# JdeRobot/slam-SDVL

Hardware: AMD Instinct MI355X
Metric: tracked frames/sec (640x480, 5-lvl pyr, ~200 feats) (higher is better)
Workload: dtype u8/f32/f64

## Files before the change

### include/sdvl_hip.h

```cpp
#ifndef SDVL_HIP_H_
#define SDVL_HIP_H_

#include <stdint.h>

#ifdef __cplusplus
extern "C" {
#endif

typedef struct sdvl_ctx sdvl_ctx;
typedef struct sdvl_frame sdvl_frame;

enum sdvl_status {
  SDVL_OK = 0,
  SDVL_ERR_INVALID = -1,
  SDVL_ERR_HIP = -2,
  SDVL_ERR_CAPACITY = -3,
  SDVL_ERR_NO_DEVICE = -4
};

#define SDVL_MAX_LEVELS 8
#define SDVL_MAX_CORNERS 6144
#define SDVL_MAX_ALIGN_FEATURES 2048
#define SDVL_CELL_KP_CAP 176
#define SDVL_MAX_CELL_SIZE 64
// ... 61 lines not shown
  int pad_;
} sdvl_search_params;

typedef struct sdvl_search_req {
  const sdvl_frame *cur;
  const sdvl_frame *ref;
  double cur_pose[7], ref_pose[7];
  double px[2];
  double bearing[3];
  double idepth, idepth_std;
  double px0[2];
  int32_t level;
  int32_t fixed;
  uint8_t desc[32];
} sdvl_search_req;

typedef struct sdvl_search_res {
  double px[2];
  int32_t found;
  int32_t level;
  int32_t best_corner;
  int32_t stage;
  int32_t lk_its;
  int32_t slevel;
} sdvl_search_res;

int sdvl_ctx_create(int device, sdvl_ctx **out);
int sdvl_ctx_destroy(sdvl_ctx *ctx);
const char *sdvl_last_error(const sdvl_ctx *ctx);
int sdvl_ctx_synchronize(sdvl_ctx *ctx);
// ... 282 lines not shown
} sdvl_track_point_stat;

int sdvl_track_create(sdvl_ctx *ctx, int n_trackers, int max_points, int max_features, int grid_cells, int max_matches,
                      int max_ransac_its, sdvl_track_set **out);
int sdvl_track_destroy(sdvl_ctx *ctx, sdvl_track_set *set);
int sdvl_frame_register(sdvl_ctx *ctx, const sdvl_frame *frame, const double *pose7);
int sdvl_frames_register(sdvl_ctx *ctx, int n, const sdvl_frame *const *frames, const double *poses7);
int sdvl_track_upload(sdvl_ctx *ctx, sdvl_track_set *set, int n, const int32_t *trackers, const int32_t *feat_buf, const int32_t *n_points,
                      const sdvl_track_point *points, const int32_t *n_features, const sdvl_track_feature *features);
int sdvl_track_append(sdvl_ctx *ctx, sdvl_track_set *set, int n, const int32_t *trackers, const int32_t *feat_buf, const int32_t *n_points,
                      const sdvl_track_point *points, const int32_t *n_features, const sdvl_track_feature *features);
int sdvl_track_align(sdvl_ctx *ctx, sdvl_track_set *set, int n_jobs, const sdvl_track_job *jobs, const uint16_t *cell_rank,
                     const int32_t *rand_raw, const sdvl_camera *cam, const sdvl_track_params *p);
int sdvl_track_search(sdvl_ctx *ctx, sdvl_track_set *set);
int sdvl_track_collect(sdvl_ctx *ctx, sdvl_track_set *set, int n_jobs, sdvl_track_result *results);
const sdvl_track_feature_out *sdvl_track_features(const sdvl_track_set *set, int job);
const sdvl_track_point_stat *sdvl_track_stats(const sdvl_track_set *set, int job);

struct sdvl_synth_view;
int sdvl_synth_render(sdvl_ctx *ctx, int n, const struct sdvl_synth_view *views, int width, int height,
                      void *dev_out, int64_t frame_bytes);
int sdvl_device_malloc(sdvl_ctx *ctx, int64_t bytes, void **out);
int sdvl_device_free(sdvl_ctx *ctx, void *p);
int sdvl_device_download(sdvl_ctx *ctx, const void *dev, int64_t bytes, void *host);
int sdvl_ctx_fork_mark(sdvl_ctx *ctx);
int sdvl_ctx_fork_begin(sdvl_ctx *ctx);
int sdvl_ctx_fork_end(sdvl_ctx *ctx);
int sdvl_host_alloc_pinned(sdvl_ctx *ctx, int64_t bytes, void **out);
int sdvl_host_free_pinned(sdvl_ctx *ctx, void *p);
int sdvl_host_register(sdvl_ctx *ctx, void *p, int64_t bytes);
// ... 7 lines not shown
```

### slam-sdvl_amd/__init__.py

```python
import ctypes as C
import os

import numpy as np

try:
    import torch
except ImportError:
    torch = None

_HERE = os.path.dirname(os.path.abspath(__file__))
CSRC = os.path.join(_HERE, "csrc")
LIB_PATH = os.path.join(CSRC, "libsdvl_hip.so")
HOST_LIB_PATH = os.path.join(_HERE, "host", "libsdvl_host.so")

SDVL_GRAY8, SDVL_RGB8, SDVL_BGR8, SDVL_RGBA8, SDVL_BGRA8 = 0, 1, 2, 3, 4

MAX_LEVELS = 8
MAX_CORNERS = 6144

u8p = C.POINTER(C.c_uint8)
i32p = C.POINTER(C.c_int32)
f64p = C.POINTER(C.c_double)
f32p = C.POINTER(C.c_float)

# ... 80 lines not shown
                ("R", C.c_double * 9), ("t", C.c_double * 3), ("plane", C.c_double * 4),
                ("seed", C.c_uint32), ("frame_id", C.c_uint32), ("texture", C.c_uint32), ("reserved_", C.c_uint32),
                ("dist", C.c_double * 5)]


ABI_SYMBOLS = [
    "sdvl_ctx_create", "sdvl_ctx_destroy", "sdvl_last_error", "sdvl_ctx_synchronize", "sdvl_ctx_stream",
    "sdvl_ctx_bind_thread", "sdvl_ctx_device", "sdvl_pointer_device", "sdvl_ctx_scratch_device",
    "sdvl_ctx_timing_enable", "sdvl_ctx_timing_only", "sdvl_ctx_timing_get", "sdvl_ctx_timing_reset",
    "sdvl_frame_create", "sdvl_frame_create_many", "sdvl_frame_destroy", "sdvl_frame_upload", "sdvl_frames_upload", "sdvl_ctx_prefetch_images", "sdvl_ctx_prefetch_fence", "sdvl_frame_set_image_device", "sdvl_frame_borrow_image_device",
    "sdvl_pyramid_build", "sdvl_frame_download_level", "sdvl_fast_num_cells", "sdvl_cell_kp_cap", "sdvl_fast_cells",
    "sdvl_detect_corners", "sdvl_frames_corner_counts", "sdvl_frame_download_corners", "sdvl_retain_best",
    "sdvl_frame_set_corners", "sdvl_frames_set_corners", "sdvl_frame_num_corners", "sdvl_shi_tomasi", "sdvl_orb_describe",
    "sdvl_frame_download_descriptors", "sdvl_filter_inputs", "sdvl_filter_inputs_begin", "sdvl_filter_inputs_end", "sdvl_filter_corners_begin", "sdvl_filter_corners_end", "sdvl_orb_describe_points", "sdvl_hamming_argmin", "sdvl_image_align", "sdvl_image_align_begin", "sdvl_image_align_end", "sdvl_align_store_create", "sdvl_align_store_destroy", "sdvl_align_store_write", "sdvl_image_align_begin_stored", "sdvl_search_points", "sdvl_search_begin", "sdvl_search_slot", "sdvl_search_run", "sdvl_align_patches", "sdvl_pose_from_matches", "sdvl_search_points_filter", "sdvl_search_run_filter", "sdvl_search_run_chain", "sdvl_search_chain_end", "sdvl_frame_footprint", "sdvl_undistort", "sdvl_frames_upload_undistorted", "sdvl_convert_gray", "sdvl_frames_upload_color", "sdvl_ctx_set_wait_hook", "sdvl_ctx_wait_done", "sdvl_ctx_wait_block", "sdvl_ctx_health", "sdvl_ctx_counters",
    "sdvl_track_create", "sdvl_track_destroy", "sdvl_frame_register", "sdvl_frames_register", "sdvl_track_upload", "sdvl_track_append", "sdvl_track_align", "sdvl_track_search",
    "sdvl_track_collect", "sdvl_track_features", "sdvl_track_stats",
    "sdvl_synth_render", "sdvl_device_malloc", "sdvl_device_free", "sdvl_device_download",
    "sdvl_frames_own_images", "sdvl_feed_create", "sdvl_feed_destroy", "sdvl_feed_last_error", "sdvl_feed_slot_arrived", "sdvl_feed_images", "sdvl_ctx_feed_acquire", "sdvl_ctx_feed_release", "sdvl_frame_footprint_cap", "sdvl_ctx_set_corner_capacity", "sdvl_frame_corner_capacity", "sdvl_detect_scratch_bytes",
    "sdvl_ctx_set_wait_spin", "sdvl_ctx_fork_mark", "sdvl_ctx_fork_begin", "sdvl_ctx_fork_end", "sdvl_host_alloc_pinned", "sdvl_host_free_pinned", "sdvl_host_register", "sdvl_host_unregister",
]

_lib = None


def load_library():
    global _lib
    if _lib is None:
        if not os.path.exists(LIB_PATH):
            raise SdvlError("libsdvl_hip.so is not built (%s): run `python -c 'import __graft_entry__ as g; g.build()'`"
                            % LIB_PATH)
        lib = C.CDLL(LIB_PATH)
# ... 551 lines not shown
```

### slam-sdvl_amd/csrc/sdvl_internal.h

```cpp
#ifndef SDVL_INTERNAL_H_
#define SDVL_INTERNAL_H_

#include <hip/hip_runtime.h>
#include <stdlib.h>
#include <hip/hip_ext.h>
#include <stdint.h>
#include <stdio.h>
#include <string.h>

#include <string>
#include <vector>

#include "../../include/sdvl_hip.h"

struct FrameView {
  uint8_t *level[SDVL_MAX_LEVELS];
  int32_t lw[SDVL_MAX_LEVELS], lh[SDVL_MAX_LEVELS];
  int32_t levels;
  int32_t n_corners;
  int32_t *corner_hdr;
  int32_t *corners;
  uint8_t *desc;
};

// ... 50 lines not shown
  void *d_detect = nullptr; size_t d_detect_bytes = 0;
  size_t pack_lds_limit = 0;
  int corner_cap = SDVL_MAX_CORNERS;
  size_t stage_off = 0;
  void *h_search = nullptr; size_t h_search_bytes = 0;
  void *d_search = nullptr; size_t d_search_bytes = 0;
  uint64_t search_busy_gen = ~0ull;
  void *d_registry = nullptr;
  int registry_cap = 0, registry_next = 0;
  std::vector<int> registry_free;
  void *d_counts = nullptr; size_t d_counts_bytes = 0;
  std::vector<sdvl_frame *> detect_frames;
  void *h_counts = nullptr; size_t h_counts_bytes = 0;
  uint64_t wait_gen = 0, counts_gen = ~0ull;
  long long counters[4] = {0, 0, 0, 0};
  std::vector<void *> slabs;
  volatile uint32_t *h_flag = nullptr;
  uint32_t flag_seq = 0;
  int wait_spin_us = 0;
  uint32_t align_ticket = 0;
  int align_pending = 0;
  uint32_t chain_ticket = 0;
  uint32_t filter_ticket = 0;
  int filter_pending = 0, filter_ccap = 0, filter_desc = 0;
  size_t filter_sc_bytes = 0, filter_row = 0;
  int chain_pending = 0;
  size_t chain_host_off = 0;
  int chain_obs_total = 0;
  void *d_nits = nullptr;
  std::vector<int32_t> nits_host;
// ... 70 lines not shown
```

### slam-sdvl_amd/csrc/sdvl_search.hip

```cpp
#include <unordered_map>
#include <utility>
#include <type_traits>
#include <vector>

#include <cmath>

#include "sdvl_internal.h"
#include "sdvl_math.h"
#include "sdvl_orb_device.h"
#include "sdvl_search_types.h"
#include "sdvl_search_prepare.h"

namespace {

using namespace sdvl;

struct PatchJob {
  const uint8_t *img;
  int w, h;
  double u, v;
};

constexpr bool kSearchOrbWindow = false, kSearchLkWindow = false;
constexpr int kLkWin = 20, kLkWinBack = 9;
// ... 203 lines not shown
#else
#define SDVL_STAT(i, v) do { } while (0)
#endif

#ifdef SDVL_SEARCH_STAMPS
__device__ unsigned long long *g_search_stamps;
constexpr int kStampRequests = 1 << 18;
#define SS_STAMP(k) do { const unsigned long long now_ = __builtin_amdgcn_s_memtime(); st_[k] += now_ - t_last_; t_last_ = now_; } while (0)
#define SS_FLUSH() do { if (lane == 0 && ri < kStampRequests && g_search_stamps) { for (int q_ = 0; q_ < 7; q_++) g_search_stamps[ri * 8 + q_] += st_[q_]; g_search_stamps[ri * 8 + 7] += 1ull; } } while (0)
#else
#define SS_STAMP(k) do { } while (0)
#define SS_FLUSH() do { } while (0)
#endif


template <bool kStage, int kW>
__global__ __launch_bounds__(64 * kW) __attribute__((amdgpu_waves_per_eu(8, 8))) void search_points_kernel(const SearchReqDev *__restrict__ reqs,
                                                                            const SearchFramePose *__restrict__ table,
                                                                            const SearchBlock *__restrict__ blocks,
                                                                            const SearchPrep *__restrict__ prep, Cam cam,
                                                                            sdvl_search_params prm, int n_blocks,
                                                                            sdvl_search_res *__restrict__ out,
                                                                            sdvl_search_res *__restrict__ out_host) {
  static_assert(kW == kWavesPerBlock || (kW == 1 && !kStage), "one wave per workgroup only without the shared corner stage");
  constexpr bool kOrbWindow = kSearchOrbWindow, kLkWindow = kSearchLkWindow;
  __shared__ WaveLds s_lds[kW];
  __shared__ uint32_t s_corners[kStage ? kLdsCorners : 1];
  const int lane = threadIdx.x & 63;
#ifdef SDVL_SEARCH_STAMPS
  unsigned long long st_[7] = {0, 0, 0, 0, 0, 0, 0}, t_last_ = __builtin_amdgcn_s_memtime();
#endif
  const int wv = kW == 1 ? static_cast<int>((blockIdx.x >> 3) % kWavesPerBlock) : __builtin_amdgcn_readfirstlane(static_cast<int>(threadIdx.x >> 6));
  const int per_xcd = static_cast<int>((kW == 1 ? gridDim.x / kWavesPerBlock : gridDim.x) >> 3);
  const int bi = static_cast<int>(blockIdx.x & 7u) * per_xcd + static_cast<int>(kW == 1 ? (blockIdx.x >> 3) / kWavesPerBlock : (blockIdx.x >> 3));
  if (bi >= n_blocks) return;
  const SearchBlock blk = blocks[bi];
  if (blk.count <= 0) return;
  const SearchFramePose &tcur = table[reqs[blk.first].cur];
  const int n_corners = min(tcur.f.n_ptr[0], SDVL_MAX_CORNERS);
  const int4 *corners_g = reinterpret_cast<const int4 *>(tcur.f.corners);
  const auto pack_corner = [](const int4 c) {
    return static_cast<uint32_t>(c.x) | (static_cast<uint32_t>(c.y) << 12) | (static_cast<uint32_t>(c.z) << 24);
  };
  const bool binned = tcur.f.bin_start != nullptr;
  if (kStage && !binned) {
    for (int ci = threadIdx.x; ci < min(n_corners, kLdsCorners); ci += 64 * kW) s_corners[ci] = pack_corner(corners_g[ci]);
    __syncthreads();
  }
  const auto corner_at = [&](int ci) { return (kStage && !binned && ci < kLdsCorners) ? s_corners[ci] : pack_corner(corners_g[ci]); };
  if (wv >= blk.count) return;
  const int ri = blk.first + wv;
  WaveLds &L = s_lds[kW == 1 ? 0 : wv];
  const SearchReqDev &rq = reqs[ri];
  const SearchFramePose &tref = table[rq.ref];
  sdvl_search_res res;
  res.px[0] = rq.px0[0];
  res.px[1] = rq.px0[1];
  res.found = 0;
  res.level = -1;
  res.best_corner = -1;
  res.stage = 0;
  res.lk_its = 0;
  res.slevel = -1;

  const int level = rq.level;
  const SearchPrep pr = prep[ri];
  if (!pr.alive) {
    if (lane == 0) { out[ri] = res; if (out_host) out_host[ri] = res; }
    return;
  }
  const auto epi = [&]() {
    const SearchPrep *pe = prep + ri;
    asm volatile("" : "+s"(pe));
    return pe;
  };
  const int slevel = pr.slevel;
  res.slevel = slevel;
  SS_STAMP(0);
  {
    const double I00 = pr.I00, I01 = pr.I01, I10 = pr.I10, I11 = pr.I11;
    const uint8_t *img = tref.f.level[level];
    const int W = tref.f.lw[level], H = tref.f.lh[level];
    const double pyrx = __builtin_ldexp(rq.px[0], -level), pyry = __builtin_ldexp(rq.px[1], -level);
    const bool bad = (I00 != I00);
// ... 230 lines not shown
  }
  SS_STAMP(2);
  res.stage = 1;
  bool matched = false;
  int best_ci = -1;
  if (best != ~0ull) {
    const int bscore = static_cast<int>(static_cast<unsigned>(best >> 20)) - 0x40000000;
    if (bscore < threshold + 1 && !(bscore >= threshold)) {
      matched = true;
      best_ci = static_cast<int>(best & 0xFFFFF);
    }
  }
  if (!matched) {
    if (lane == 0) { out[ri] = res; if (out_host) out_host[ri] = res; }
    SS_FLUSH();
    return;
  }
  res.best_corner = best_ci;
  const uint32_t bpk = best_pk;
  const int bx = static_cast<int>(bpk & 0xFFFu), by = static_cast<int>((bpk >> 12) & 0xFFFu), bl = static_cast<int>(bpk >> 24);
  const double mpx = static_cast<double>(bx * (1 << bl)), mpy = static_cast<double>(by * (1 << bl));
  res.px[0] = mpx;
  res.px[1] = mpy;
  float u = static_cast<float>(__builtin_ldexp(mpx, -slevel)), v = static_cast<float>(__builtin_ldexp(mpy, -slevel));
  int its = 0;
  const bool conv = kLkWindow ? align_patch_wave<true>(L, tcur.f.level[slevel], tcur.f.lw[slevel], tcur.f.lh[slevel], prm.max_align_its, lane, &u, &v,
                                                       &its, prm.lk_tree_sums != 0)
                              : align_patch_wave<false>(L, tcur.f.level[slevel], tcur.f.lw[slevel], tcur.f.lh[slevel], prm.max_align_its, lane, &u, &v,
                                                        &its, prm.lk_tree_sums != 0);
  SS_STAMP(4);
#ifdef SDVL_SEARCH_STAMPS
  st_[5] += its;
#endif
  res.lk_its = its;
  res.stage = 2;
  if (conv) {
    res.px[0] = static_cast<double>(u) * (1 << slevel);
    res.px[1] = static_cast<double>(v) * (1 << slevel);
    res.level = slevel;
    res.found = 1;
    res.stage = 3;
  }
  if (lane == 0) { out[ri] = res; if (out_host) out_host[ri] = res; }
  SS_FLUSH();
}

#ifdef SDVL_SEARCH_STAMPS
extern "C" int sdvl_debug_search_stamps(unsigned long long *out8, int reset) {
  static unsigned long long *d_buf = nullptr;
  const size_t bytes = sizeof(unsigned long long) * 8 * kStampRequests;
  if (reset) {
    if (!d_buf && hipMalloc(&d_buf, bytes) != hipSuccess) return -1;
    if (hipMemset(d_buf, 0, bytes) != hipSuccess) return -1;
    return hipMemcpyToSymbol(HIP_SYMBOL(g_search_stamps), &d_buf, sizeof(d_buf)) == hipSuccess ? 0 : -1;
  }
  if (!d_buf) return -1;
  std::vector<unsigned long long> h(static_cast<size_t>(8) * kStampRequests);
  if (hipMemcpy(h.data(), d_buf, bytes, hipMemcpyDeviceToHost) != hipSuccess) return -1;
  for (int q = 0; q < 8; q++) out8[q] = 0;
// ... 277 lines not shown
#ifdef SDVL_SEARCH_STATS
  {
    static int launches = 0;
    if (++launches % 200 == 0) {
      unsigned long long h[8];
      if (hipMemcpyFromSymbol(h, HIP_SYMBOL(g_search_stats), sizeof(h)) == hipSuccess)
        fprintf(stderr, "search stats after %d launches: requests %llu, binned %llu, full scans %llu (frame binned %llu, line ok %llu), scan rounds %llu, corners in range %llu\n",
                launches, h[0], h[1], h[2], h[6], h[7], h[3], h[4]);
    }
  }
#endif
  SDVL_HIP_CHECK(ctx, hipGetLastError());
  return SDVL_OK;
}

int sdvl_select_matches_launch(sdvl_ctx *ctx, int n_frames, const ChainFrameDev *d_frames, const int32_t *d_cand_req,
                               const int32_t *d_cand_first, const sdvl_search_res *d_res, const double *d_req_point,
                               const sdvl_camera *cam, PoseJobDev *d_jobs, sdvl_pose_obs *d_obs, int32_t *d_nobs, int32_t *d_match_cand) {
  if (n_frames <= 0) return SDVL_OK;
  Cam c{cam->width, cam->height, cam->fx, cam->fy, cam->u0, cam->v0};
  SDVL_LAUNCH(ctx, "select_matches", select_matches_kernel, dim3(n_frames), dim3(256), d_frames, d_cand_req, d_cand_first, d_res, d_req_point, c,
              d_jobs, d_obs, d_nobs, d_match_cand);
  SDVL_HIP_CHECK(ctx, hipGetLastError());
  return SDVL_OK;
}

extern "C" {

static_assert(sizeof(sdvl_search_req_packed) == sizeof(SearchReqDev), "public and device request records are one layout");

// ... 403 lines not shown
```

### slam-sdvl_amd/csrc/sdvl_search_types.h

```cpp
#ifndef SDVL_SEARCH_TYPES_H_
#define SDVL_SEARCH_TYPES_H_

#include "sdvl_internal.h"
#include "sdvl_math.h"

constexpr int kWavesPerBlock = 4;
constexpr int kLdsCorners = 4096;

struct SearchBlock {
  int first, count;
};

struct SearchFrame {
  const uint8_t *level[SDVL_MAX_LEVELS];
  int lw[SDVL_MAX_LEVELS], lh[SDVL_MAX_LEVELS];
  const int32_t *corners;
  const uint8_t *desc;
  const int32_t *n_ptr;
  int levels;
  int bin_gw;
  const int32_t *bin_start;
  const uint2 *bin_entries;
  int bin_cells, pad_;
  int pad2_[2];
};

// ... 65 lines not shown
  int cur_id, last_id;
  int frame_id, max_matches;
  int n_feat, n_points;
  double last_pose[7];
  double pad_;
  const uint8_t *last_level[SDVL_MAX_LEVELS];
  double T0[7];
  double pad2_;
};

extern "C" TrackPoint *sdvl_track_points_device(sdvl_track_set *set, int *max_points, int *n_trackers);

int sdvl_search_launch_device(sdvl_ctx *ctx, int n_slots, const SearchReqDev *d_reqs, const SearchFramePose *d_table,
                              const SearchBlock *d_blocks, int n_blocks, const sdvl_camera *cam, const sdvl_search_params *p,
                              SearchPrep *d_prep, sdvl_search_res *d_res, sdvl_search_res *h_res, bool prepared = false);
int sdvl_select_matches_launch(sdvl_ctx *ctx, int n_frames, const ChainFrameDev *d_frames, const int32_t *d_cand_req,
                               const int32_t *d_cand_first, const sdvl_search_res *d_res, const double *d_req_point,
                               const sdvl_camera *cam, PoseJobDev *d_jobs, sdvl_pose_obs *d_obs, int32_t *d_nobs, int32_t *d_match_cand);
int sdvl_image_align_track_enqueue(sdvl_ctx *ctx, int n_jobs, const TrackJobDev *d_jobs, const TrackPoint *d_points, const TrackFeat *d_feats0,
                                   const TrackFeat *d_feats1, int np, int nfeat_cap, int max_nf, int levels, const sdvl_camera *cam,
                                   const sdvl_align_params *p, sdvl_align_result *d_results, int batch_size);
extern "C" int sdvl_ensure_nits_table(sdvl_ctx *ctx, int npoints_cfg, int max_its, int max_size);

#endif
```

### slam-sdvl_amd/csrc/sdvl_track.hip

```cpp
#include <atomic>
#include <chrono>
#include <vector>

#include "sdvl_internal.h"
#include "sdvl_math.h"
#include "sdvl_search_types.h"
#include "sdvl_search_prepare.h"

namespace {

using namespace sdvl;


struct UploadRec {
  int tracker, feat_buf;
  int n_points, n_feat;
  long long point_off, feat_off;
  int point_dst, feat_dst;
  long long pad_;
};

struct RegisterRec {
  SearchFramePose e;
  int id, pad_;
// ... 46 lines not shown
  const int fw = r.n_feat * static_cast<int>(sizeof(TrackFeat) / 16);
  for (int i = threadIdx.x; i < fw; i += 256) df[i] = sf[i];
}

constexpr int kProjThreads = 512;

__global__ __launch_bounds__(kProjThreads) void track_project_kernel(const TrackJobDev *__restrict__ jobs, TrackPoint *__restrict__ points,
                                                                     const TrackFeat *__restrict__ feats0, const TrackFeat *__restrict__ feats1,
                                                                     int np, int nf, int stride, int mm, int max_its,
                                                                     const sdvl_align_result *__restrict__ ares,
                                                                     const uint16_t *__restrict__ cell_rank, int cells, Cam cam, int cell_size,
                                                                     int patch, SearchFramePose *__restrict__ registry,
                                                                     SearchReqDev *__restrict__ reqs, double *__restrict__ req_point,
                                                                     int32_t *__restrict__ cand_first, int32_t *__restrict__ cand_feat,
                                                                     SearchBlock *__restrict__ blocks, ChainFrameDev *__restrict__ chain,
                                                                     sdvl_search_params sprm, SearchPrep *__restrict__ prep) {
  extern __shared__ __attribute__((aligned(16))) uint8_t s_dyn[];
  unsigned long long *s_key = reinterpret_cast<unsigned long long *>(s_dyn);
  double *s_px = reinterpret_cast<double *>(s_key + stride);
  uint16_t *s_cell = reinterpret_cast<uint16_t *>(s_px + 2 * static_cast<size_t>(stride));
  __shared__ double s_pose[7];
  __shared__ int s_ncand;
  const int j = blockIdx.x, tid = threadIdx.x;
  const TrackJobDev &jb = jobs[j];
  const TrackFeat *F = (jb.feat_buf ? feats1 : feats0) + static_cast<size_t>(jb.tracker) * nf;
  TrackPoint *P = points + static_cast<size_t>(jb.tracker) * np;
  const int n_feat = jb.n_feat;
  const int base = j * stride;
  if (tid == 0) {
    const Rigid pose = se3_mul(se3_from7(ares[j].T), se3_from7(jb.last_pose));
    se3_to7(pose, s_pose);
// ... 60 lines not shown
    for (int w = 0; w < 8; w++) rq.desc[w] = p.desc[w];
    reqs[base + r] = rq;
    if (prep) prep[base + r] = search_prepare_one(rq, pose, se3_from7(registry[p.ref].pose), cam, sprm, &jb.cur);
    double *rp = req_point + 3 * static_cast<size_t>(base + r);
    rp[0] = p.P[0]; rp[1] = p.P[1]; rp[2] = p.P[2];
    cand_feat[base + r] = i;
    s_cell[r] = static_cast<uint16_t>(key >> 48);
  }
  __syncthreads();
  for (int k = tid; k < stride; k += static_cast<int>(blockDim.x)) {
    if (k < n_cand) {
      int first = k;
      const uint16_t c = s_cell[k];
      while (first > 0 && s_cell[first - 1] == c) first--;
      cand_first[base + k] = base + first;
    } else {
      reqs[base + k].level = -1;
      if (prep) {
        prep[base + k].alive = 0;
        prep[base + k].slevel = -1;
      }
    }
  }
  const int nblk = stride / kWavesPerBlock;
  for (int b = tid; b < nblk; b += static_cast<int>(blockDim.x)) {
    int cnt = n_cand - b * kWavesPerBlock;
    cnt = cnt < 0 ? 0 : (cnt > kWavesPerBlock ? kWavesPerBlock : cnt);
    blocks[j * nblk + b] = SearchBlock{base + b * kWavesPerBlock, cnt};
  }
  if (tid == 0) {
    ChainFrameDev c;
// ... 181 lines not shown
  int n, np, nf, cells, mm, max_its;
  TrackPoint *d_points = nullptr;
  TrackFeat *d_feats[2] = {nullptr, nullptr};
  uint8_t *d_scratch = nullptr;
  size_t scratch_bytes = 0;
  TrackJobDev *d_jobs;
  uint16_t *d_cell_rank;
  int32_t *d_rand;
  sdvl_align_result *d_ares;
  SearchReqDev *d_reqs;
  SearchPrep *d_prep;
  sdvl_search_res *d_res;
  double *d_reqpt;
  int32_t *d_cfirst, *d_cfeat;
  SearchBlock *d_blocks;
  ChainFrameDev *d_chain;
  PoseJobDev *d_pjobs;
  sdvl_pose_obs *d_obs;
  void *d_hyp;
  sdvl_pose_result *d_pres;
  int32_t *d_lists, *d_nobs;
  uint8_t *h_pinned = nullptr;
  sdvl_track_result *h_results;
  sdvl_track_feature_out *h_feats;
  sdvl_track_point_stat *h_stats;
  std::vector<int> n_points;
  std::vector<int> n_feat[2];
  std::vector<sdvl_track_job> jobs;
  int stride = 0;
  int phase = 0;
  uint32_t ticket = 0;
  sdvl_camera cam;
  sdvl_track_params prm;
};

namespace {
template <typename T>
T *carve(uint8_t *&p, size_t count) {
  T *r = reinterpret_cast<T *>(p);
  p += (sizeof(T) * count + 255) / 256 * 256;
  return r;
}
}

extern "C" {

int sdvl_track_create(sdvl_ctx *ctx, int n, int max_points, int max_features, int grid_cells, int max_matches, int max_ransac_its,
                      sdvl_track_set **out) {
// ... 1 lines not shown
  *out = nullptr;
  SDVL_REQUIRE(ctx, n >= 1 && n <= 65536, "tracker count out of range");
  SDVL_REQUIRE(ctx, max_points >= 1 && max_points < SDVL_TRACK_DUPLICATE && max_features >= 4 && max_features <= 4096, "table capacities out of range (features <= 4096)");
  SDVL_REQUIRE(ctx, grid_cells >= 1 && grid_cells <= 65535, "grid too large");
  SDVL_REQUIRE(ctx, max_matches >= 1 && max_matches <= 1024 && max_matches <= max_features, "max_matches outside the device pose stage's range (1024)");
  SDVL_REQUIRE(ctx, max_ransac_its >= 1 && max_ransac_its <= 4096, "bad max_ransac_its");
  SDVL_HIP_CHECK(ctx, sdvl_bind_device(ctx));
  sdvl_track_set *s = new sdvl_track_set();
  s->ctx = ctx;
  s->n = n;
  s->np = max_points;
  s->nf = (max_features + 3) / 4 * 4;
  s->cells = grid_cells;
  s->mm = max_matches;
  s->max_its = max_ransac_its;
  const size_t N = static_cast<size_t>(n), NF = N * s->nf;
  hipError_t e = hipMalloc(reinterpret_cast<void **>(&s->d_points), sizeof(TrackPoint) * N * s->np);
  if (e == hipSuccess) e = hipMalloc(reinterpret_cast<void **>(&s->d_feats[0]), sizeof(TrackFeat) * NF);
  if (e == hipSuccess) e = hipMalloc(reinterpret_cast<void **>(&s->d_feats[1]), sizeof(TrackFeat) * NF);
  for (int pass = 0; pass < 2 && e == hipSuccess; pass++) {
    uint8_t *p = pass ? s->d_scratch : nullptr;
    s->d_jobs = carve<TrackJobDev>(p, N);
    s->d_cell_rank = carve<uint16_t>(p, N * s->cells);
    s->d_rand = carve<int32_t>(p, N * s->max_its);
    s->d_ares = carve<sdvl_align_result>(p, N);
    s->d_reqs = carve<SearchReqDev>(p, NF);
    s->d_prep = carve<SearchPrep>(p, NF);
    s->d_res = carve<sdvl_search_res>(p, NF);
    s->d_reqpt = carve<double>(p, NF * 3);
    s->d_cfirst = carve<int32_t>(p, NF);
    s->d_cfeat = carve<int32_t>(p, NF);
    s->d_blocks = carve<SearchBlock>(p, NF / kWavesPerBlock);
    s->d_chain = carve<ChainFrameDev>(p, N);
    s->d_pjobs = carve<PoseJobDev>(p, N);
    s->d_obs = carve<sdvl_pose_obs>(p, N * s->mm);
    s->d_hyp = carve<uint8_t>(p, sdvl_pose_hyp_bytes() * N * s->max_its);
    s->d_pres = carve<sdvl_pose_result>(p, N);
    s->d_lists = carve<int32_t>(p, N * s->mm);
    s->d_nobs = carve<int32_t>(p, N);
    if (!pass) {
      s->scratch_bytes = reinterpret_cast<size_t>(p);
      e = hipMalloc(reinterpret_cast<void **>(&s->d_scratch), s->scratch_bytes);
    }
  }
  if (e == hipSuccess) {
    const size_t hb = (sizeof(sdvl_track_result) * N + 255) / 256 * 256, fb = (sizeof(sdvl_track_feature_out) * NF + 255) / 256 * 256;
    const size_t sb = sizeof(sdvl_track_point_stat) * N * s->np;
// ... 1 lines not shown
    if (e == hipSuccess) {
      memset(s->h_pinned, 0, hb + fb + sb);
      s->h_results = reinterpret_cast<sdvl_track_result *>(s->h_pinned);
      s->h_feats = reinterpret_cast<sdvl_track_feature_out *>(s->h_pinned + hb);
      s->h_stats = reinterpret_cast<sdvl_track_point_stat *>(s->h_pinned + hb + fb);
    }
  }
  if (e != hipSuccess) {
    ctx->err = std::string("sdvl_track_create: ") + hipGetErrorString(e);
    sdvl_track_destroy(ctx, s);
    return SDVL_ERR_HIP;
  }
  s->n_points.assign(n, 0);
  s->n_feat[0].assign(n, 0);
  s->n_feat[1].assign(n, 0);
  *out = s;
  return SDVL_OK;
}

TrackPoint *sdvl_track_points_device(sdvl_track_set *set, int *max_points, int *n_trackers) {
  if (max_points) *max_points = set->np;
  if (n_trackers) *n_trackers = set->n;
  return set->d_points;
}

int sdvl_track_destroy(sdvl_ctx *ctx, sdvl_track_set *s) {
  if (!ctx || !s) return SDVL_ERR_INVALID;
  (void)sdvl_bind_device(ctx);
  (void)sdvl_stream_wait(ctx);
  if (s->d_points) (void)hipFree(s->d_points);
  if (s->d_feats[0]) (void)hipFree(s->d_feats[0]);
  if (s->d_feats[1]) (void)hipFree(s->d_feats[1]);
  if (s->d_scratch) (void)hipFree(s->d_scratch);
  if (s->h_pinned) (void)hipHostFree(s->h_pinned);
  delete s;
  return SDVL_OK;
}

int sdvl_frame_register(sdvl_ctx *ctx, const sdvl_frame *f, const double *pose7) { return sdvl_frames_register(ctx, 1, &f, pose7); }

int sdvl_frames_register(sdvl_ctx *ctx, int n, const sdvl_frame *const *frames, const double *poses7) {
  if (!ctx || n < 0 || (n > 0 && (!frames || !poses7))) return SDVL_ERR_INVALID;
  if (n == 0) return SDVL_OK;
  for (int i = 0; i < n; i++)
    SDVL_REQUIRE(ctx, frames[i] && frames[i]->home == ctx && frames[i]->reg_id >= 0 && frames[i]->reg_id < ctx->registry_cap,
                 "frame was not created on this context");
  void *hs = nullptr, *dsx = nullptr;
  int rc = sdvl_stage_alloc(ctx, sizeof(RegisterRec) * static_cast<size_t>(n), &hs, &dsx);
  if (rc) return rc;
// ... 187 lines not shown
      SDVL_HIP_CHECK(ctx, hipFuncSetAttribute(reinterpret_cast<const void *>(track_project_kernel), hipFuncAttributeMaxDynamicSharedMemorySize,
                                              4096 * (8 + 16 + 2) + 64));
      attr_devices.fetch_or(bit, std::memory_order_release);
    }
  }
  {
    const size_t lds = static_cast<size_t>(stride) * (8 + 16 + 2) + 64;
    hipEvent_t ev_a = nullptr, ev_b = nullptr;
    sdvl_timer_events(ctx, "track_project", &ev_a, &ev_b);
    const int proj_threads = stride <= 256 ? (s->n > 32 ? 128 : 256) : kProjThreads;
    hipExtLaunchKernelGGL(track_project_kernel, dim3(n_jobs), dim3(proj_threads), lds, ctx->stream, ev_a, ev_b, 0,
                          static_cast<const TrackJobDev *>(s->d_jobs), s->d_points, static_cast<const TrackFeat *>(s->d_feats[0]),
                          static_cast<const TrackFeat *>(s->d_feats[1]), s->np, s->nf, stride, s->mm, s->max_its,
                          static_cast<const sdvl_align_result *>(s->d_ares), static_cast<const uint16_t *>(s->d_cell_rank), s->cells, c,
                          s->prm.cell_size, s->prm.patch_size, registry, s->d_reqs, s->d_reqpt, s->d_cfirst, s->d_cfeat, s->d_blocks, s->d_chain,
                          s->prm.search, s->d_prep);
    SDVL_HIP_CHECK(ctx, hipGetLastError());
  }
  int rc = sdvl_search_launch_device(ctx, n_jobs * stride, s->d_reqs, registry, s->d_blocks, n_jobs * (stride / kWavesPerBlock), &s->cam,
                                     &s->prm.search, s->d_prep, s->d_res, nullptr,  true);
  if (rc) return rc;
  rc = sdvl_select_matches_launch(ctx, n_jobs, s->d_chain, nullptr, s->d_cfirst, s->d_res, s->d_reqpt, &s->cam, s->d_pjobs, s->d_obs, s->d_nobs,
                                  nullptr);
  if (rc) return rc;
  sdvl_pose_params pp = s->prm.pose;
  pp.pad_ = 1;
  rc = sdvl_pose_enqueue_device(ctx, n_jobs, s->d_pjobs, s->d_obs, s->d_rand, static_cast<const int32_t *>(ctx->d_nits), &pp, s->d_hyp, s->d_pres,
                                s->d_lists, s->mm, s->n);
  if (rc) return rc;
  {
    const size_t lds = (static_cast<size_t>(stride + 1) * 2 + stride + 64 + 7) / 8 * 8 + static_cast<size_t>(s->mm) * 8;
    hipEvent_t ev_a = nullptr, ev_b = nullptr;
    sdvl_timer_events(ctx, "track_commit", &ev_a, &ev_b);
    hipExtLaunchKernelGGL(track_commit_kernel, dim3(n_jobs), dim3(256), lds, ctx->stream, ev_a, ev_b, 0, static_cast<const TrackJobDev *>(s->d_jobs),
                          s->d_points, static_cast<const TrackFeat *>(s->d_feats[0]), static_cast<const TrackFeat *>(s->d_feats[1]), s->d_feats[0],
// ... 12 lines not shown
int sdvl_track_collect(sdvl_ctx *ctx, sdvl_track_set *s, int n_jobs, sdvl_track_result *results) {
  if (!ctx || !s || s->ctx != ctx || !results) return SDVL_ERR_INVALID;
  SDVL_REQUIRE(ctx, s->phase == 2 && n_jobs == static_cast<int>(s->jobs.size()), "sdvl_track_collect without a matching sdvl_track_search");
  SDVL_HIP_CHECK(ctx, sdvl_mark_wait(ctx, SDVL_MARK_CHAIN, s->ticket));
  s->phase = 0;
  memcpy(results, s->h_results, sizeof(sdvl_track_result) * n_jobs);
  for (int j = 0; j < n_jobs; j++) {
    const sdvl_track_job &a = s->jobs[j];
    s->n_feat[1 - a.feat_buf][a.tracker] = results[j].matches;
    if (results[j].n_corners >= 0) a.cur->v.n_corners = results[j].n_corners;
  }
  ctx->wait_gen++;
  return SDVL_OK;
}

const sdvl_track_feature_out *sdvl_track_features(const sdvl_track_set *s, int job) {
  return (s && job >= 0 && job < s->n) ? s->h_feats + static_cast<size_t>(job) * s->nf : nullptr;
}

const sdvl_track_point_stat *sdvl_track_stats(const sdvl_track_set *s, int job) {
  return (s && job >= 0 && job < s->n) ? s->h_stats + static_cast<size_t>(job) * s->np : nullptr;
}

}
```

Before: 459,500.

## Search each grid cell's candidates sequentially in one wave, stopping at first match

The projection kernel now emits per-cell runs of candidate requests. A new search kernel assigns one wave per run and walks the candidates in order, breaking at the first converged match. It marks the remaining candidates as not tried instead of searching every candidate in parallel, which is meant to skip redundant searches whose results the per-cell match selection would discard. In exchange, work within a cell becomes serialised, and the kernel gives up the multi-wave blocks with the shared LDS corner stage. It is enabled only when there are more than 32 trackers, and an environment variable can turn it off. Host mirror and cell-inspection APIs are also added for checking results.

```diff
diff --git a/include/sdvl_hip.h b/include/sdvl_hip.h
--- a/include/sdvl_hip.h
+++ b/include/sdvl_hip.h
@@ -99,6 +99,8 @@
   int32_t fixed;
   uint8_t desc[32];
 } sdvl_search_req;
+
+#define SDVL_SEARCH_NOT_TRIED 4
 
 typedef struct sdvl_search_res {
   double px[2];
@@ -411,6 +413,8 @@
                      const int32_t *rand_raw, const sdvl_camera *cam, const sdvl_track_params *p);
 int sdvl_track_search(sdvl_ctx *ctx, sdvl_track_set *set);
 int sdvl_track_collect(sdvl_ctx *ctx, sdvl_track_set *set, int n_jobs, sdvl_track_result *results);
+int sdvl_track_search_mirror(sdvl_ctx *ctx, sdvl_track_set *set, int fill_byte, const sdvl_search_res **out, int *stride);
+int sdvl_track_search_cells(sdvl_ctx *ctx, sdvl_track_set *set, int job, int cap, int32_t *cand_first, int32_t *n_cand);
 const sdvl_track_feature_out *sdvl_track_features(const sdvl_track_set *set, int job);
 const sdvl_track_point_stat *sdvl_track_stats(const sdvl_track_set *set, int job);
 
diff --git a/slam-sdvl_amd/__init__.py b/slam-sdvl_amd/__init__.py
--- a/slam-sdvl_amd/__init__.py
+++ b/slam-sdvl_amd/__init__.py
@@ -118,7 +118,7 @@
     "sdvl_frame_set_corners", "sdvl_frames_set_corners", "sdvl_frame_num_corners", "sdvl_shi_tomasi", "sdvl_orb_describe",
     "sdvl_frame_download_descriptors", "sdvl_filter_inputs", "sdvl_filter_inputs_begin", "sdvl_filter_inputs_end", "sdvl_filter_corners_begin", "sdvl_filter_corners_end", "sdvl_orb_describe_points", "sdvl_hamming_argmin", "sdvl_image_align", "sdvl_image_align_begin", "sdvl_image_align_end", "sdvl_align_store_create", "sdvl_align_store_destroy", "sdvl_align_store_write", "sdvl_image_align_begin_stored", "sdvl_search_points", "sdvl_search_begin", "sdvl_search_slot", "sdvl_search_run", "sdvl_align_patches", "sdvl_pose_from_matches", "sdvl_search_points_filter", "sdvl_search_run_filter", "sdvl_search_run_chain", "sdvl_search_chain_end", "sdvl_frame_footprint", "sdvl_undistort", "sdvl_frames_upload_undistorted", "sdvl_convert_gray", "sdvl_frames_upload_color", "sdvl_ctx_set_wait_hook", "sdvl_ctx_wait_done", "sdvl_ctx_wait_block", "sdvl_ctx_health", "sdvl_ctx_counters",
     "sdvl_track_create", "sdvl_track_destroy", "sdvl_frame_register", "sdvl_frames_register", "sdvl_track_upload", "sdvl_track_append", "sdvl_track_align", "sdvl_track_search",
-    "sdvl_track_collect", "sdvl_track_features", "sdvl_track_stats",
+    "sdvl_track_collect", "sdvl_track_features", "sdvl_track_stats", "sdvl_track_search_mirror", "sdvl_track_search_cells",
     "sdvl_synth_render", "sdvl_device_malloc", "sdvl_device_free", "sdvl_device_download",
     "sdvl_frames_own_images", "sdvl_feed_create", "sdvl_feed_destroy", "sdvl_feed_last_error", "sdvl_feed_slot_arrived", "sdvl_feed_images", "sdvl_ctx_feed_acquire", "sdvl_ctx_feed_release", "sdvl_frame_footprint_cap", "sdvl_ctx_set_corner_capacity", "sdvl_frame_corner_capacity", "sdvl_detect_scratch_bytes",
     "sdvl_ctx_set_wait_spin", "sdvl_ctx_fork_mark", "sdvl_ctx_fork_begin", "sdvl_ctx_fork_end", "sdvl_host_alloc_pinned", "sdvl_host_free_pinned", "sdvl_host_register", "sdvl_host_unregister",
diff --git a/slam-sdvl_amd/csrc/sdvl_internal.h b/slam-sdvl_amd/csrc/sdvl_internal.h
--- a/slam-sdvl_amd/csrc/sdvl_internal.h
+++ b/slam-sdvl_amd/csrc/sdvl_internal.h
@@ -88,6 +88,7 @@
   void *h_counts = nullptr; size_t h_counts_bytes = 0;
   uint64_t wait_gen = 0, counts_gen = ~0ull;
   long long counters[4] = {0, 0, 0, 0};
+  sdvl_track_set *last_track_set = nullptr;
   std::vector<void *> slabs;
   volatile uint32_t *h_flag = nullptr;
   uint32_t flag_seq = 0;
diff --git a/slam-sdvl_amd/csrc/sdvl_search.hip b/slam-sdvl_amd/csrc/sdvl_search.hip
--- a/slam-sdvl_amd/csrc/sdvl_search.hip
+++ b/slam-sdvl_amd/csrc/sdvl_search.hip
@@ -241,43 +241,20 @@
 #endif
 
 
-template <bool kStage, int kW>
-__global__ __launch_bounds__(64 * kW) __attribute__((amdgpu_waves_per_eu(8, 8))) void search_points_kernel(const SearchReqDev *__restrict__ reqs,
-                                                                            const SearchFramePose *__restrict__ table,
-                                                                            const SearchBlock *__restrict__ blocks,
-                                                                            const SearchPrep *__restrict__ prep, Cam cam,
-                                                                            sdvl_search_params prm, int n_blocks,
-                                                                            sdvl_search_res *__restrict__ out,
-                                                                            sdvl_search_res *__restrict__ out_host) {
-  static_assert(kW == kWavesPerBlock || (kW == 1 && !kStage), "one wave per workgroup only without the shared corner stage");
+template <bool kStage>
+__device__ __forceinline__ bool search_request(const SearchReqDev *__restrict__ reqs, const SearchFramePose *__restrict__ table,
+                                               const SearchPrep *__restrict__ prep, const sdvl_search_params &prm, const SearchFramePose &tcur,
+                                               const uint32_t *s_corners, const bool binned, const int n_corners, const int ri, const int lane,
+                                               WaveLds &L, sdvl_search_res *__restrict__ out, sdvl_search_res *__restrict__ out_host) {
   constexpr bool kOrbWindow = kSearchOrbWindow, kLkWindow = kSearchLkWindow;
-  __shared__ WaveLds s_lds[kW];
-  __shared__ uint32_t s_corners[kStage ? kLdsCorners : 1];
-  const int lane = threadIdx.x & 63;
 #ifdef SDVL_SEARCH_STAMPS
   unsigned long long st_[7] = {0, 0, 0, 0, 0, 0, 0}, t_last_ = __builtin_amdgcn_s_memtime();
 #endif
-  const int wv = kW == 1 ? static_cast<int>((blockIdx.x >> 3) % kWavesPerBlock) : __builtin_amdgcn_readfirstlane(static_cast<int>(threadIdx.x >> 6));
-  const int per_xcd = static_cast<int>((kW == 1 ? gridDim.x / kWavesPerBlock : gridDim.x) >> 3);
-  const int bi = static_cast<int>(blockIdx.x & 7u) * per_xcd + static_cast<int>(kW == 1 ? (blockIdx.x >> 3) / kWavesPerBlock : (blockIdx.x >> 3));
-  if (bi >= n_blocks) return;
-  const SearchBlock blk = blocks[bi];
-  if (blk.count <= 0) return;
-  const SearchFramePose &tcur = table[reqs[blk.first].cur];
-  const int n_corners = min(tcur.f.n_ptr[0], SDVL_MAX_CORNERS);
   const int4 *corners_g = reinterpret_cast<const int4 *>(tcur.f.corners);
   const auto pack_corner = [](const int4 c) {
     return static_cast<uint32_t>(c.x) | (static_cast<uint32_t>(c.y) << 12) | (static_cast<uint32_t>(c.z) << 24);
   };
-  const bool binned = tcur.f.bin_start != nullptr;
-  if (kStage && !binned) {
-    for (int ci = threadIdx.x; ci < min(n_corners, kLdsCorners); ci += 64 * kW) s_corners[ci] = pack_corner(corners_g[ci]);
-    __syncthreads();
-  }
   const auto corner_at = [&](int ci) { return (kStage && !binned && ci < kLdsCorners) ? s_corners[ci] : pack_corner(corners_g[ci]); };
-  if (wv >= blk.count) return;
-  const int ri = blk.first + wv;
-  WaveLds &L = s_lds[kW == 1 ? 0 : wv];
   const SearchReqDev &rq = reqs[ri];
   const SearchFramePose &tref = table[rq.ref];
   sdvl_search_res res;
@@ -294,7 +271,7 @@
   const SearchPrep pr = prep[ri];
   if (!pr.alive) {
     if (lane == 0) { out[ri] = res; if (out_host) out_host[ri] = res; }
-    return;
+    return false;
   }
   const auto epi = [&]() {
     const SearchPrep *pe = prep + ri;
@@ -555,7 +532,7 @@
   if (!matched) {
     if (lane == 0) { out[ri] = res; if (out_host) out_host[ri] = res; }
     SS_FLUSH();
-    return;
+    return false;
   }
   res.best_corner = best_ci;
   const uint32_t bpk = best_pk;
@@ -584,6 +561,79 @@
   }
   if (lane == 0) { out[ri] = res; if (out_host) out_host[ri] = res; }
   SS_FLUSH();
+  return conv;
+}
+
+template <bool kStage, int kW>
+__global__ __launch_bounds__(64 * kW) __attribute__((amdgpu_waves_per_eu(8, 8))) void search_points_kernel(const SearchReqDev *__restrict__ reqs,
+                                                                            const SearchFramePose *__restrict__ table,
+                                                                            const SearchBlock *__restrict__ blocks,
+                                                                            const SearchPrep *__restrict__ prep, Cam cam,
+                                                                            sdvl_search_params prm, int n_blocks,
+                                                                            sdvl_search_res *__restrict__ out,
+                                                                            sdvl_search_res *__restrict__ out_host) {
+  static_assert(kW == kWavesPerBlock || (kW == 1 && !kStage), "one wave per workgroup only without the shared corner stage");
+  __shared__ WaveLds s_lds[kW];
+  __shared__ uint32_t s_corners[kStage ? kLdsCorners : 1];
+  const int lane = threadIdx.x & 63;
+  const int wv = kW == 1 ? static_cast<int>((blockIdx.x >> 3) % kWavesPerBlock) : __builtin_amdgcn_readfirstlane(static_cast<int>(threadIdx.x >> 6));
+  const int per_xcd = static_cast<int>((kW == 1 ? gridDim.x / kWavesPerBlock : gridDim.x) >> 3);
+  const int bi = static_cast<int>(blockIdx.x & 7u) * per_xcd + static_cast<int>(kW == 1 ? (blockIdx.x >> 3) / kWavesPerBlock : (blockIdx.x >> 3));
+  if (bi >= n_blocks) return;
+  const SearchBlock blk = blocks[bi];
+  if (blk.count <= 0) return;
+  const SearchFramePose &tcur = table[reqs[blk.first].cur];
+  const int n_corners = min(tcur.f.n_ptr[0], SDVL_MAX_CORNERS);
+  const bool binned = tcur.f.bin_start != nullptr;
+  if (kStage && !binned) {
+    const int4 *corners_g = reinterpret_cast<const int4 *>(tcur.f.corners);
+    for (int ci = threadIdx.x; ci < min(n_corners, kLdsCorners); ci += 64 * kW) {
+      const int4 c = corners_g[ci];
+      s_corners[ci] = static_cast<uint32_t>(c.x) | (static_cast<uint32_t>(c.y) << 12) | (static_cast<uint32_t>(c.z) << 24);
+    }
+    __syncthreads();
+  }
+  if (wv >= blk.count) return;
+  (void)search_request<kStage>(reqs, table, prep, prm, tcur, s_corners, binned, n_corners, blk.first + wv, lane, s_lds[kW == 1 ? 0 : wv], out, out_host);
+}
+
+__global__ __launch_bounds__(64) __attribute__((amdgpu_waves_per_eu(8, 8))) void search_cell_runs_kernel(const SearchReqDev *__restrict__ reqs,
+                                                                            const SearchFramePose *__restrict__ table,
+                                                                            const SearchRun *__restrict__ runs,
+                                                                            const SearchPrep *__restrict__ prep, sdvl_search_params prm,
+                                                                            int n_runs, sdvl_search_res *__restrict__ out,
+                                                                            sdvl_search_res *__restrict__ out_host) {
+  __shared__ WaveLds s_lds[1];
+  const int lane = threadIdx.x;
+  const int per_xcd = static_cast<int>(gridDim.x >> 3);
+  const int k = static_cast<int>(blockIdx.x & 7u) * per_xcd + static_cast<int>(blockIdx.x >> 3);
+  if (k >= n_runs) return;
+  const SearchRun run = runs[k];
+  if (run.len <= 0) return;
+  const SearchFramePose &tcur = table[reqs[run.first].cur];
+  const int n_corners = min(tcur.f.n_ptr[0], SDVL_MAX_CORNERS);
+  const bool binned = tcur.f.bin_start != nullptr;
+  const int end = run.first + run.len;
+  int ri = run.first;
+#pragma unroll 1
+  for (; ri < end; ri++) {
+    const bool found = search_request<false>(reqs, table, prep, prm, tcur, nullptr, binned, n_corners, ri, lane, s_lds[0], out, out_host);
+    if (__builtin_amdgcn_readfirstlane(found ? 1 : 0)) break;
+    wave_sync();
+  }
+  for (int q = ri + 1 + lane; q < end; q += 64) {
+    sdvl_search_res res;
+    res.px[0] = reqs[q].px0[0];
+    res.px[1] = reqs[q].px0[1];
+    res.found = 0;
+    res.level = -1;
+    res.best_corner = -1;
+    res.stage = SDVL_SEARCH_NOT_TRIED;
+    res.lk_its = 0;
+    res.slevel = -1;
+    out[q] = res;
+    if (out_host) out_host[q] = res;
+  }
 }
 
 #ifdef SDVL_SEARCH_STAMPS
@@ -891,6 +941,18 @@
   return SDVL_OK;
 }
 
+int sdvl_search_launch_runs_device(sdvl_ctx *ctx, int n_runs, const SearchReqDev *d_reqs, const SearchFramePose *d_table, const SearchRun *d_runs,
+                                   const sdvl_search_params *p, const SearchPrep *d_prep, sdvl_search_res *d_res, sdvl_search_res *h_res) {
+  SDVL_REQUIRE(ctx, p->patch_size == 8, "only patch_size 8 is supported (one wave64 per 8x8 patch)");
+  SDVL_REQUIRE(ctx, p->max_fast_levels >= 1 && p->max_fast_levels <= 4, "bad max_fast_levels");
+  SDVL_REQUIRE(ctx, p->max_align_its >= 0 && p->margin >= 4, "bad max_align_its / margin");
+  if (n_runs <= 0) return SDVL_OK;
+  SDVL_LAUNCH(ctx, "search_points", search_cell_runs_kernel, dim3(static_cast<unsigned>((n_runs + 7) / 8 * 8)), dim3(64), d_reqs, d_table, d_runs, d_prep,
+              *p, n_runs, d_res, h_res);
+  SDVL_HIP_CHECK(ctx, hipGetLastError());
+  return SDVL_OK;
+}
+
 int sdvl_select_matches_launch(sdvl_ctx *ctx, int n_frames, const ChainFrameDev *d_frames, const int32_t *d_cand_req,
                                const int32_t *d_cand_first, const sdvl_search_res *d_res, const double *d_req_point,
                                const sdvl_camera *cam, PoseJobDev *d_jobs, sdvl_pose_obs *d_obs, int32_t *d_nobs, int32_t *d_match_cand) {
diff --git a/slam-sdvl_amd/csrc/sdvl_search_types.h b/slam-sdvl_amd/csrc/sdvl_search_types.h
--- a/slam-sdvl_amd/csrc/sdvl_search_types.h
+++ b/slam-sdvl_amd/csrc/sdvl_search_types.h
@@ -10,6 +10,11 @@
 struct SearchBlock {
   int first, count;
 };
+
+struct SearchRun {
+  int first, len;
+};
+constexpr int kSearchRunMinSet = 32;
 
 struct SearchFrame {
   const uint8_t *level[SDVL_MAX_LEVELS];
@@ -105,6 +110,8 @@
 int sdvl_search_launch_device(sdvl_ctx *ctx, int n_slots, const SearchReqDev *d_reqs, const SearchFramePose *d_table,
                               const SearchBlock *d_blocks, int n_blocks, const sdvl_camera *cam, const sdvl_search_params *p,
                               SearchPrep *d_prep, sdvl_search_res *d_res, sdvl_search_res *h_res, bool prepared = false);
+int sdvl_search_launch_runs_device(sdvl_ctx *ctx, int n_runs, const SearchReqDev *d_reqs, const SearchFramePose *d_table, const SearchRun *d_runs,
+                                   const sdvl_search_params *p, const SearchPrep *d_prep, sdvl_search_res *d_res, sdvl_search_res *h_res);
 int sdvl_select_matches_launch(sdvl_ctx *ctx, int n_frames, const ChainFrameDev *d_frames, const int32_t *d_cand_req,
                                const int32_t *d_cand_first, const sdvl_search_res *d_res, const double *d_req_point,
                                const sdvl_camera *cam, PoseJobDev *d_jobs, sdvl_pose_obs *d_obs, int32_t *d_nobs, int32_t *d_match_cand);
diff --git a/slam-sdvl_amd/csrc/sdvl_track.hip b/slam-sdvl_amd/csrc/sdvl_track.hip
--- a/slam-sdvl_amd/csrc/sdvl_track.hip
+++ b/slam-sdvl_amd/csrc/sdvl_track.hip
@@ -84,7 +84,8 @@
                                                                      SearchReqDev *__restrict__ reqs, double *__restrict__ req_point,
                                                                      int32_t *__restrict__ cand_first, int32_t *__restrict__ cand_feat,
                                                                      SearchBlock *__restrict__ blocks, ChainFrameDev *__restrict__ chain,
-                                                                     sdvl_search_params sprm, SearchPrep *__restrict__ prep) {
+                                                                     sdvl_search_params sprm, SearchPrep *__restrict__ prep,
+                                                                     SearchRun *__restrict__ runs) {
   extern __shared__ __attribute__((aligned(16))) uint8_t s_dyn[];
   unsigned long long *s_key = reinterpret_cast<unsigned long long *>(s_dyn);
   double *s_px = reinterpret_cast<double *>(s_key + stride);
@@ -175,7 +176,14 @@
       const uint16_t c = s_cell[k];
       while (first > 0 && s_cell[first - 1] == c) first--;
       cand_first[base + k] = base + first;
+      if (runs) {
+        int len = 0;
+        if (first == k)
+          for (len = 1; k + len < n_cand && s_cell[k + len] == c;) len++;
+        runs[base + k] = SearchRun{base + k, len};
+      }
     } else {
+      if (runs) runs[base + k] = SearchRun{base + k, 0};
       reqs[base + k].level = -1;
       if (prep) {
         prep[base + k].alive = 0;
@@ -387,6 +395,7 @@
   double *d_reqpt;
   int32_t *d_cfirst, *d_cfeat;
   SearchBlock *d_blocks;
+  SearchRun *d_runs;
   ChainFrameDev *d_chain;
   PoseJobDev *d_pjobs;
   sdvl_pose_obs *d_obs;
@@ -405,6 +414,8 @@
   uint32_t ticket = 0;
   sdvl_camera cam;
   sdvl_track_params prm;
+  bool cell_runs = false;
+  sdvl_search_res *h_search_res = nullptr;
 };
 
 namespace {
@@ -436,6 +447,7 @@
   s->cells = grid_cells;
   s->mm = max_matches;
   s->max_its = max_ransac_its;
+  s->cell_runs = n > kSearchRunMinSet && getenv("SDVL_SEARCH_PER_REQUEST") == nullptr;
   const size_t N = static_cast<size_t>(n), NF = N * s->nf;
   hipError_t e = hipMalloc(reinterpret_cast<void **>(&s->d_points), sizeof(TrackPoint) * N * s->np);
   if (e == hipSuccess) e = hipMalloc(reinterpret_cast<void **>(&s->d_feats[0]), sizeof(TrackFeat) * NF);
@@ -453,6 +465,7 @@
     s->d_cfirst = carve<int32_t>(p, NF);
     s->d_cfeat = carve<int32_t>(p, NF);
     s->d_blocks = carve<SearchBlock>(p, NF / kWavesPerBlock);
+    s->d_runs = carve<SearchRun>(p, NF);
     s->d_chain = carve<ChainFrameDev>(p, N);
     s->d_pjobs = carve<PoseJobDev>(p, N);
     s->d_obs = carve<sdvl_pose_obs>(p, N * s->mm);
@@ -484,6 +497,7 @@
   s->n_points.assign(n, 0);
   s->n_feat[0].assign(n, 0);
   s->n_feat[1].assign(n, 0);
+  ctx->last_track_set = s;
   *out = s;
   return SDVL_OK;
 }
@@ -498,11 +512,13 @@
   if (!ctx || !s) return SDVL_ERR_INVALID;
   (void)sdvl_bind_device(ctx);
   (void)sdvl_stream_wait(ctx);
+  if (ctx->last_track_set == s) ctx->last_track_set = nullptr;
   if (s->d_points) (void)hipFree(s->d_points);
   if (s->d_feats[0]) (void)hipFree(s->d_feats[0]);
   if (s->d_feats[1]) (void)hipFree(s->d_feats[1]);
   if (s->d_scratch) (void)hipFree(s->d_scratch);
   if (s->h_pinned) (void)hipHostFree(s->h_pinned);
+  if (s->h_search_res) (void)hipHostFree(s->h_search_res);
   delete s;
   return SDVL_OK;
 }
@@ -720,11 +736,17 @@
                           static_cast<const TrackFeat *>(s->d_feats[1]), s->np, s->nf, stride, s->mm, s->max_its,
                           static_cast<const sdvl_align_result *>(s->d_ares), static_cast<const uint16_t *>(s->d_cell_rank), s->cells, c,
                           s->prm.cell_size, s->prm.patch_size, registry, s->d_reqs, s->d_reqpt, s->d_cfirst, s->d_cfeat, s->d_blocks, s->d_chain,
-                          s->prm.search, s->d_prep);
+                          s->prm.search, s->d_prep, s->cell_runs ? s->d_runs : nullptr);
     SDVL_HIP_CHECK(ctx, hipGetLastError());
   }
-  int rc = sdvl_search_launch_device(ctx, n_jobs * stride, s->d_reqs, registry, s->d_blocks, n_jobs * (stride / kWavesPerBlock), &s->cam,
-                                     &s->prm.search, s->d_prep, s->d_res, nullptr,  true);
+  int rc;
+  if (s->cell_runs) {
+    ctx->counters[3]++;
+    rc = sdvl_search_launch_runs_device(ctx, n_jobs * stride, s->d_reqs, registry, s->d_runs, &s->prm.search, s->d_prep, s->d_res, s->h_search_res);
+  } else {
+    rc = sdvl_search_launch_device(ctx, n_jobs * stride, s->d_reqs, registry, s->d_blocks, n_jobs * (stride / kWavesPerBlock), &s->cam,
+                                   &s->prm.search, s->d_prep, s->d_res, s->h_search_res,  true);
+  }
   if (rc) return rc;
   rc = sdvl_select_matches_launch(ctx, n_jobs, s->d_chain, nullptr, s->d_cfirst, s->d_res, s->d_reqpt, &s->cam, s->d_pjobs, s->d_obs, s->d_nobs,
                                   nullptr);
@@ -767,6 +789,41 @@
   return SDVL_OK;
 }
 
+int sdvl_track_search_mirror(sdvl_ctx *ctx, sdvl_track_set *s, int fill_byte, const sdvl_search_res **out, int *stride) {
+  if (ctx && !s) s = ctx->last_track_set;
+  if (!ctx || !s || s->ctx != ctx || !out) return SDVL_ERR_INVALID;
+  SDVL_REQUIRE(ctx, s->phase == 0 || s->phase == 1, "sdvl_track_search_mirror between sdvl_track_search and sdvl_track_collect");
+  const size_t bytes = sizeof(sdvl_search_res) * static_cast<size_t>(s->n) * s->nf;
+  SDVL_HIP_CHECK(ctx, sdvl_bind_device(ctx));
+  if (!s->h_search_res) {
+    SDVL_HIP_CHECK(ctx, hipHostMalloc(reinterpret_cast<void **>(&s->h_search_res), bytes, hipHostMallocDefault));
+    memset(s->h_search_res, 0, bytes);
+  }
+  if (fill_byte >= 0) {
+    memset(s->h_search_res, fill_byte, bytes);
+    SDVL_HIP_CHECK(ctx, hipMemsetAsync(s->d_res, fill_byte, bytes, ctx->stream));
+  }
+  *out = s->h_search_res;
+  if (stride) *stride = s->stride;
+  return SDVL_OK;
+}
+
+int sdvl_track_search_cells(sdvl_ctx *ctx, sdvl_track_set *s, int job, int cap, int32_t *cand_first, int32_t *n_cand) {
+  if (ctx && !s) s = ctx->last_track_set;
+  if (!ctx || !s || s->ctx != ctx || !cand_first || !n_cand || cap < 0) return SDVL_ERR_INVALID;
+  SDVL_REQUIRE(ctx, s->phase == 0 && job >= 0 && job < static_cast<int>(s->jobs.size()), "sdvl_track_search_cells: no collected step holds this job");
+  SDVL_HIP_CHECK(ctx, sdvl_bind_device(ctx));
+  SDVL_HIP_CHECK(ctx, sdvl_stream_wait(ctx));
+  ChainFrameDev fr;
+  SDVL_HIP_CHECK(ctx, hipMemcpy(&fr, s->d_chain + job, sizeof(fr), hipMemcpyDeviceToHost));
+  const int n = fr.cand_end - fr.cand_begin;
+  *n_cand = n;
+  const int m = n < cap ? n : cap;
+  if (m > 0) SDVL_HIP_CHECK(ctx, hipMemcpy(cand_first, s->d_cfirst + fr.cand_begin, sizeof(int32_t) * m, hipMemcpyDeviceToHost));
+  for (int k = 0; k < m; k++) cand_first[k] -= fr.cand_begin;
+  return SDVL_OK;
+}
+
 const sdvl_track_feature_out *sdvl_track_features(const sdvl_track_set *s, int job) {
   return (s && job >= 0 && job < s->n) ? s->h_feats + static_cast<size_t>(job) * s->nf : nullptr;
 }
```

Result: slower. 364,600 (-20.7%).
